# ChuhanZhou/News_Recommendation_Model

Measured on AMD Instinct MI355X. Metric: train impressions/sec, higher is better.
Workload: dtype f32

## Files before the change

### include/nrm_hotpath.h

```cpp
#ifndef NRM_HOTPATH_H
#define NRM_HOTPATH_H

#ifdef __cplusplus
extern "C" {
#endif

#define NRM_ABI_VERSION 7
#define NRM_OK 0
#define NRM_EINVAL (-1)
#define NRM_ELAUNCH (-2)

typedef void* nrm_stream_t;

int nrm_abi_version(void);
const char* nrm_last_error(void);
int nrm_build_flags(void);
const char* nrm_source_digest(void);
const char* nrm_build_info(void);


#define NRM_MMA_F32 0
#define NRM_MMA_BF16 1
#define NRM_MMA_BF16X3 2
long nrm_pwattn_packed_floats(int D);
// ... 42 lines not shown
int nrm_gemm_tn_nsplit(int ncols_i, int ncols_j, int R, int mma);
int nrm_gemm_tn(const float* A, int lda, int ncols_i, const float* B, int ldb, int ncols_j, int R,
                float* ws, int ldws, float* colsum, float* zero_out, long zero_n, int mma, nrm_stream_t stream);

int nrm_slab_reduce(const float* ws, int nsplit, int nj, int ldws, int ni, float* out, long out_istride, long out_jstride,
                    float* out2, long out2_istride, long out2_jstride, float sign2,
                    const float* vec, float* vec_out, nrm_stream_t stream);
typedef struct nrm_slab_desc {
    const float* ws; int nsplit, nj, ldws, ni;
    float* out; long out_istride, out_jstride;
    float* out2; long out2_istride, out2_jstride; float sign2;
    const float* vec; float* vec_out;
} nrm_slab_desc;
int nrm_slab_reduce_multi(const nrm_slab_desc* descs, int n, nrm_stream_t stream);

int nrm_colreduce(int mode, const float* x, const float* dy, const float* mean, const float* rstd,
                  float* s0, float* s1, int R, int N, int ld, nrm_stream_t stream);
int nrm_bn_finalize(int stage, const float* s, float* out, float* running, int R, int N, float momentum, float eps,
                    nrm_stream_t stream);
int nrm_mul_bwd(const float* dy, int lddy, const float* g, int ldg, const float* e, int lde, float* dg, float* de, int ldo,
                int R, int N, nrm_stream_t stream);
int nrm_bn_apply(const float* x, const float* mean, const float* rstd, const float* gamma, const float* beta,
                 float* y, int R, int N, int ld, nrm_stream_t stream);
int nrm_bn_backward(const float* x, const float* dy, const float* mean, const float* rstd, const float* gamma,
                    const float* s0, const float* s1, const float* add, float* dx, int R, int N, int ld, int training,
                    nrm_stream_t stream);
int nrm_concat_cols(const float* const* srcs, const long* lds, const int* widths, int n, float* out, int ldo, long R,
                    nrm_stream_t stream);

int nrm_pool_bmm(const float* W, long wsb, long wsi, long wsj, const float* X, int ldx, float* out,
// ... 60 lines not shown
```

### news_recommendation_model_amd/csrc/capi.hip

```cpp
#include <stdarg.h>
#include <stdint.h>
#include <stdio.h>
#include <stdlib.h>
#include <vector>

#include "../../include/nrm_hotpath.h"
#include "pwattn.hpp"
#include "gemm.hpp"
#include "head.hpp"
#include "pool_loss.hpp"
#include "frontend.hpp"
#include "scoring.hpp"
#include "compact.hpp"

static thread_local char g_err[512] = "";

static int fail(int code, const char* fmt, ...) {
    va_list ap;
    va_start(ap, fmt);
    vsnprintf(g_err, sizeof(g_err), fmt, ap);
    va_end(ap);
    return code;
}
static int check_hip(hipError_t e, const char* what) {
// ... 338 lines not shown
    if (n == 0) return NRM_OK;
    std::vector<nrm::SlabReduceParams> ps((size_t)n);
    for (int i = 0; i < n; ++i) {
        const nrm_slab_desc& d = descs[i];
        if (!d.ws || !d.out) return fail(NRM_EINVAL, "nrm_slab_reduce_multi: entry %d: null pointer", i);
        if (d.nsplit <= 0 || d.nj <= 0 || d.ni <= 0 || d.ldws < d.ni)
            return fail(NRM_EINVAL, "nrm_slab_reduce_multi: entry %d: nsplit=%d nj=%d ni=%d ldws=%d", i, d.nsplit, d.nj, d.ni, d.ldws);
        if ((d.vec == nullptr) != (d.vec_out == nullptr)) return fail(NRM_EINVAL, "nrm_slab_reduce_multi: entry %d: vec and vec_out go together", i);
        nrm::SlabReduceParams& p = ps[(size_t)i];
        p.ws = d.ws; p.nsplit = d.nsplit; p.nj = d.nj; p.ldws = d.ldws; p.ni = d.ni; p.out = d.out; p.ors = d.out_istride; p.ocs = d.out_jstride;
        p.out2 = d.out2; p.ors2 = d.out2_istride; p.ocs2 = d.out2_jstride; p.sign2 = d.sign2; p.vec = d.vec; p.vec_out = d.vec_out;
    }
    return check_hip(nrm::slab_reduce_multi_launch(ps.data(), n, (hipStream_t)stream), "slab_reduce_multi");
}

static int check_bn(const char* fn, int R, int N, int ld) {
    if (R < 0 || N <= 0 || N % 4 || ld % 4 || ld < N) return fail(NRM_EINVAL, "%s: R=%d N=%d ld=%d (N, ld multiples of 4)", fn, R, N, ld);
    return NRM_OK;
}

int nrm_colreduce(int mode, const float* x, const float* dy, const float* mean, const float* rstd,
                  float* s0, float* s1, int R, int N, int ld, nrm_stream_t stream) {
    if (int rc = check_bn("nrm_colreduce", R, N, ld)) return rc;
    if (!x || !s0 || (mode >= 1 && !mean) || (mode == 2 && (!dy || !rstd || !s1)) || mode < 0 || mode > 2)
        return fail(NRM_EINVAL, "nrm_colreduce: bad argument for mode %d", mode);
    return check_hip(nrm::colred_launch(mode, x, dy, mean, rstd, s0, s1, R, N, ld, (hipStream_t)stream), "colreduce");
}

int nrm_bn_finalize(int stage, const float* s, float* out, float* running, int R, int N, float momentum, float eps,
                    nrm_stream_t stream) {
// ... 265 lines not shown
```

### news_recommendation_model_amd/csrc/head.hip

```cpp
#include "common.hpp"
#include "head.hpp"

namespace nrm {

template <int MODE>
__global__ __launch_bounds__(256) void colred_kernel(const float* __restrict__ x, const float* __restrict__ dy,
                                                     const float* __restrict__ mean, const float* __restrict__ rstd,
                                                     float* __restrict__ s0, float* __restrict__ s1,
                                                     int R, int N, int ld, int rpb) {
    __shared__ f32x4 red[2][8][32];
    const int tx = threadIdx.x, ty = threadIdx.y;
    const int col = blockIdx.x * 128 + 4 * tx;
    const bool cok = col < N;
    f32x4 a0 = f32x4{0.f, 0.f, 0.f, 0.f}, a1 = a0, mu = a0, rs = a0;
    if (cok && MODE >= 1) mu = *reinterpret_cast<const f32x4*>(mean + col);
    if (cok && MODE == 2) rs = *reinterpret_cast<const f32x4*>(rstd + col);
    const int r_lo = blockIdx.y * rpb, r_hi = min(R, r_lo + rpb);
    if (cok) {
        for (int r = r_lo + ty; r < r_hi; r += 8) {
            const f32x4 xv = *reinterpret_cast<const f32x4*>(x + (size_t)r * ld + col);
            if (MODE == 0) a0 += xv;
            else if (MODE == 1) { const f32x4 d = xv - mu; a0 += d * d; }
            else {
                const f32x4 g = *reinterpret_cast<const f32x4*>(dy + (size_t)r * ld + col);
// ... 240 lines not shown
    else          hipLaunchKernelGGL(small_linear_relu_fwd_kernel<float>, grid, dim3(256), 0, st, (const float*)x, w, b, y, R, K, N, ldy);
    return hipGetLastError();
}

hipError_t small_linear_relu_bwd_launch(const void* x, int x_is_f64, const float* w, const float* b, const float* dy, int lddy,
                                        long R, int K, int N, float* dwb, hipStream_t st) {
    if (R <= 0) return hipSuccess;
    if (K < 1 || K > SL_KMAX || N < 1 || N > SL_NMAX || lddy < N) return hipErrorInvalidValue;
    long blocks = (R + 255) / 256;
    if (blocks > 256) blocks = 256;
    if (x_is_f64) hipLaunchKernelGGL(small_linear_relu_bwd_kernel<double>, dim3((unsigned)blocks), dim3(256), 0, st, (const double*)x, w, b, dy, lddy, R, K, N, dwb);
    else          hipLaunchKernelGGL(small_linear_relu_bwd_kernel<float>, dim3((unsigned)blocks), dim3(256), 0, st, (const float*)x, w, b, dy, lddy, R, K, N, dwb);
    return hipGetLastError();
}

}
```

### news_recommendation_model_amd/csrc/head.hpp

```cpp
#pragma once
#include <hip/hip_runtime.h>

namespace nrm {
hipError_t colred_launch(int mode, const float* x, const float* dy, const float* mean, const float* rstd,
                         float* s0, float* s1, int R, int N, int ld, hipStream_t st);
hipError_t bn_apply_launch(const float* x, const float* mean, const float* rstd, const float* gamma, const float* beta,
                           float* y, long R, int N, int ld, hipStream_t st);
hipError_t bn_bwd_launch(const float* x, const float* dy, const float* mean, const float* rstd, const float* gamma,
                         const float* s0, const float* s1, const float* add, float* dx, long R, int N, int ld, int training,
                         hipStream_t st);
constexpr int CONCAT_MAX = 8;
struct ConcatTable { const float* src[CONCAT_MAX]; long ld[CONCAT_MAX]; int start[CONCAT_MAX]; int n; };
hipError_t concat_cols_launch(const ConcatTable& tab, float* out, long R, int ldo, int total, hipStream_t st);
hipError_t bn_finalize_launch(int stage, const float* s, float* out, float* running, int R, int N, float momentum, float eps,
                              hipStream_t st);
hipError_t mul_bwd_launch(const float* dy, const float* g, const float* e, float* dg, float* de, long R, int N,
                          int lddy, int ldg, int lde, int ldo, hipStream_t st);
hipError_t small_linear_relu_fwd_launch(const void* x, int x_is_f64, const float* w, const float* b, float* y, long R, int K, int N,
                                        int ldy, hipStream_t st);
hipError_t small_linear_relu_bwd_launch(const void* x, int x_is_f64, const float* w, const float* b, const float* dy, int lddy,
                                        long R, int K, int N, float* dwb, hipStream_t st);
}
```

### news_recommendation_model_amd/modules.py

```python
from __future__ import annotations

import os

import torch
import torch.nn as nn
import torch.nn.functional as F

from . import ops
from .config import Dims, TIME_TABLE_ROWS, model_config

_ACTIVATIONS = {
    "relu": nn.ReLU, "gelu": nn.GELU, "tanh": nn.Tanh, "sigmoid": nn.Sigmoid,
    "leaky_relu": nn.LeakyReLU, "elu": nn.ELU,
}


class MLP(nn.Module):

    def __init__(self, input_dim, output_dim, activation_type="gelu"):
        super().__init__()
        self.fc1 = nn.Linear(input_dim, input_dim // 4)
        self.fc2 = nn.Linear(input_dim // 4, output_dim)
        self.activation_type = activation_type
        self.activation = _ACTIVATIONS.get(str(activation_type).lower(), nn.GELU)()
# ... 158 lines not shown
class UserModel(nn.Module):

    def __init__(self, user_num=0):
        super().__init__()
        self.invariant_interest_model = UserInvariantInterestModel()
        self.instant_interest_model = UserInstantInterestModel(8)
        width = (sum(self.invariant_interest_model.embed_setting) + model_config["pca_vector"]) * 2 \
            + self.instant_interest_model.output_dim
        self.bn = nn.BatchNorm1d(width)
        self.gate = MLP(width, width)
        self.mlp = MLP(width, width)
        self.out_mlp = MLP(width, 1)
        self.delta = nn.Parameter(torch.zeros(user_num + 1))
        self.bce_loss = nn.BCELoss()
        self.softmax = nn.Softmax(dim=1)

    def forward(self, x_history, x_target, x_global):
        inv = self.invariant_interest_model
        if type(inv) is UserInvariantInterestModel and not (inv._forward_hooks or inv._forward_pre_hooks):
            pooled_lab, pooled_ti, lab_t, ti_t = inv.forward_parts(x_history, x_target)
            eu_L = self.instant_interest_model(x_global)
            e = ops.concat_last((pooled_lab, pooled_ti, eu_L, lab_t, ti_t))
        else:
            eu_H, ec = inv(x_history, x_target)
            eu_L = self.instant_interest_model(x_global)
            e = ops.concat_last((eu_H, eu_L, ec))
        B, T, N = e.shape
        rows = e.reshape(B * T, N)
        g = self.gate
        if isinstance(g.activation, nn.GELU) and g.activation.approximate == "none":
            gated = ops.gate_block(rows, self.bn, g.fc1.weight, g.fc1.bias, g.fc2.weight, g.fc2.bias)
        else:
            gated = g.forward_times(ops.batch_norm(rows, self.bn), rows)
        return self.out_mlp(self.mlp(gated)).reshape(B, T)

    def forward_compact(self, x_history, xt_compact, xg_compact, plan):
        if self.training:
            raise RuntimeError("UserModel.forward_compact is inference only: call .eval() first (training-mode BatchNorm takes its "
                               "statistics over the rows of the launch, and the compact path drops the padded ones)")
        inv = self.invariant_interest_model
        ops._require_gpu(x_history, xt_compact, xg_compact)
        B, H, N = x_history.shape[0], x_history.shape[1], xt_compact.shape[0]
        if plan.B != B or plan.N != N or xg_compact.shape[0] != N:
            raise RuntimeError(f"forward_compact: plan for {plan.B} impressions / {plan.N} rows, got {B} / {N} target and {xg_compact.shape[0]} global rows")
        if B * H == 0 or N == 0:
            raise RuntimeError("cannot reshape tensor of 0 elements (empty batch / history / candidate list)")
        for att in (inv.label_attention, inv.text_img_attention):
            mlp = getattr(att, "mlp", None)
            if not (type(att) is PointwiseAttentionExpanded and isinstance(mlp, MLP) and isinstance(mlp.activation, nn.GELU)
# ... 8 lines not shown
            lab_h, ti_h = ops.frontend(x_history, True, d.n_subcat, d.pca_vector, *tables)
            lab_t, ti_t = ops.frontend(xt_compact.unsqueeze(0), False, d.n_subcat, d.pca_vector, *tables)
            lab_h = ops.linear(lab_h, inv.w1.weight, inv.w1.bias)
            pooled = []
            for att, t, h in ((inv.label_attention, lab_t[0], lab_h), (inv.text_img_attention, ti_t[0], ti_h)):
                m = att.mlp
                pooled.append(ops.attend_pool_ragged(t, h, m.fc1.weight, m.fc1.bias, m.fc2.weight, m.fc2.bias, tabs["cand_imp"],
                                                     tabs["cand_off"], plan.max_count, mma=att.mma))
            eu_L = self.instant_interest_model(xg_compact)
            rows = ops.concat_last((pooled[0], pooled[1], eu_L, lab_t[0], ti_t[0]))
            g = self.gate
            if isinstance(g.activation, nn.GELU) and g.activation.approximate == "none":
                gated = ops.gate_block(rows, self.bn, g.fc1.weight, g.fc1.bias, g.fc2.weight, g.fc2.bias)
            else:
                gated = g.forward_times(ops.batch_norm(rows, self.bn), rows)
            return self.out_mlp(self.mlp(gated)).reshape(N)

    def loss(self, id, out, label, alpha=0.95):
        return ops.softmax_bce_loss(out, self.delta, label, id, alpha)
```

### news_recommendation_model_amd/native.py

```python
from __future__ import annotations

import ctypes
import os
import threading

_HERE = os.path.dirname(os.path.abspath(__file__))
LIB_PATH = os.environ.get("NRM_HOTPATH_LIB") or os.path.join(_HERE, "libnrm_hotpath.so")
ABI_VERSION = 7

_c_fp = ctypes.c_void_p
_c_i, _c_l = ctypes.c_int, ctypes.c_long

SIGNATURES = {
    "nrm_abi_version": (_c_i, []),
    "nrm_last_error": (ctypes.c_char_p, []),
    "nrm_build_flags": (_c_i, []),
    "nrm_source_digest": (ctypes.c_char_p, []),
    "nrm_build_info": (ctypes.c_char_p, []),
    "nrm_pwattn_packed_floats": (_c_l, [_c_i]),
    "nrm_pwattn_pack_wp": (_c_i, [_c_fp, _c_i, _c_i, _c_i, _c_fp, _c_fp]),
    "nrm_pwattn_fwd": (_c_i, [_c_fp] * 9 + [_c_i] * 5 + [_c_fp]),
    "nrm_pwattn_bwd_dz": (_c_i, [_c_fp] * 7 + [_c_i] * 5 + [_c_fp]),
    "nrm_pwattn_bwd_rw_supported": (_c_i, [_c_i, _c_i]),
    "nrm_pwattn_bwd_rw_packed_floats": (_c_l, [_c_i, _c_i]),
# ... 5 lines not shown
    "nrm_pwattn_bwd_dp_dtdh": (_c_i, [_c_fp] * 6 + [_c_i] * 4 + [_c_fp]),
    "nrm_pwattn_bwd_nsplit": (_c_i, [_c_i] * 5),
    "nrm_pwattn_bwd_contract": (_c_i, [_c_fp] * 4 + [_c_i] + [_c_fp] * 3 + [_c_i] * 7 + [_c_fp]),
    "nrm_gemm_packed_floats": (_c_l, [_c_i, _c_i, _c_i]),
    "nrm_gemm_nt_bf16_supported": (_c_i, [_c_i, _c_i, _c_i]),
    "nrm_gemm_pack": (_c_i, [_c_fp, _c_l, _c_l, _c_i, _c_i, _c_fp, _c_fp]),
    "nrm_gemm_nt": (_c_i, [_c_fp, _c_i, _c_i, _c_fp, _c_i, _c_i, _c_fp, _c_fp, _c_i, _c_fp, _c_i, _c_fp, _c_i, _c_i, _c_i, _c_fp]),
    "nrm_slab_reduce": (_c_i, [_c_fp, _c_i, _c_i, _c_i, _c_i, _c_fp, _c_l, _c_l, _c_fp, _c_l, _c_l, ctypes.c_float,
                               _c_fp, _c_fp, _c_fp]),
    "nrm_bn_finalize": (_c_i, [_c_i, _c_fp, _c_fp, _c_fp, _c_i, _c_i, ctypes.c_float, ctypes.c_float, _c_fp]),
    "nrm_mul_bwd": (_c_i, [_c_fp, _c_i, _c_fp, _c_i, _c_fp, _c_i, _c_fp, _c_fp, _c_i, _c_i, _c_i, _c_fp]),
    "nrm_gemm_tn_nsplit": (_c_i, [_c_i, _c_i, _c_i, _c_i]),
    "nrm_gemm_tn": (_c_i, [_c_fp, _c_i, _c_i, _c_fp, _c_i, _c_i, _c_i, _c_fp, _c_i, _c_fp, _c_fp, _c_l, _c_i, _c_fp]),
    "nrm_gemm_pack_multi": (_c_i, [_c_fp, _c_i, _c_fp]),
    "nrm_slab_reduce_multi": (_c_i, [_c_fp, _c_i, _c_fp]),
    "nrm_colreduce": (_c_i, [_c_i] + [_c_fp] * 6 + [_c_i] * 3 + [_c_fp]),
    "nrm_bn_apply": (_c_i, [_c_fp] * 6 + [_c_i] * 3 + [_c_fp]),
    "nrm_bn_backward": (_c_i, [_c_fp] * 9 + [_c_i] * 4 + [_c_fp]),
    "nrm_concat_cols": (_c_i, [_c_fp, _c_fp, _c_fp, _c_i, _c_fp, _c_i, _c_l, _c_fp]),
    "nrm_pool_bmm": (_c_i, [_c_fp, _c_l, _c_l, _c_l, _c_fp, _c_i, _c_fp] + [_c_i] * 5 + [_c_fp]),
    "nrm_pool_rowdot": (_c_i, [_c_fp, _c_i, _c_fp, _c_fp] + [_c_i] * 4 + [_c_fp, _c_i, _c_fp]),
    "nrm_small_linear_relu_fwd": (_c_i, [_c_fp, _c_i, _c_fp, _c_fp, _c_fp, _c_l, _c_i, _c_i, _c_i, _c_fp]),
    "nrm_small_linear_relu_bwd": (_c_i, [_c_fp, _c_i, _c_fp, _c_fp, _c_fp, _c_i, _c_l, _c_i, _c_i, _c_fp, _c_fp]),
    "nrm_loss_fwd_bwd": (_c_i, [_c_fp, _c_i, _c_fp, _c_i, _c_fp, _c_fp, _c_l, ctypes.c_float, _c_i, _c_i, _c_fp, _c_fp, _c_i, _c_fp, _c_fp, _c_fp]),
    "nrm_adam_step": (_c_i, [_c_fp] * 4 + [_c_l] + [ctypes.c_float] * 5 + [_c_i, _c_i, _c_fp]),
    "nrm_adam_step_dev": (_c_i, [_c_fp] * 4 + [_c_l] + [ctypes.c_float] * 5 + [_c_fp, _c_i, _c_fp]),
    "nrm_gather_flat": (_c_i, [_c_fp, _c_fp, _c_fp, _c_i, _c_fp, _c_l, _c_fp]),
    "nrm_row_auc": (_c_i, [_c_fp] * 3 + [_c_i, _c_i] + [_c_fp] * 3),
    "nrm_ensemble_rank_max_candidates": (_c_i, []),
    "nrm_ensemble_rank": (_c_i, [_c_fp] * 3 + [_c_i, _c_fp, _c_fp, _c_i, _c_i] + [_c_fp] * 5),
# ... 97 lines not shown
```

### news_recommendation_model_amd/ops.py

```python
from __future__ import annotations

import torch

from . import native

EPI_BIAS, EPI_GELU, EPI_DGELU, EPI_MUL = 0, 1, 2, 3
MMA_F32, MMA_BF16, MMA_BF16X3 = 0, 1, 2
DZ_F32, DZ_HL4 = 0, 1
_MMA_NAMES = {"f32": MMA_F32, "fp32": MMA_F32, "float32": MMA_F32, "bf16": MMA_BF16, "bfloat16": MMA_BF16, "bf16x3": MMA_BF16X3}
_default_mma = MMA_F32


def resolve_mma(mma):
    if mma is None:
        return _default_mma
    if isinstance(mma, str):
        if mma.lower() not in _MMA_NAMES:
            raise ValueError(f"attention arithmetic {mma!r}: expected 'f32', 'bf16' or 'bf16x3'")
        return _MMA_NAMES[mma.lower()]
    if int(mma) not in (MMA_F32, MMA_BF16, MMA_BF16X3):
        raise ValueError(f"attention arithmetic {mma!r}: expected NRM_MMA_F32 (0), NRM_MMA_BF16 (1) or NRM_MMA_BF16X3 (2)")
    return int(mma)


# ... 109 lines not shown
    return ctypes.cast(ctypes.pointer(desc_or_array), ctypes.c_void_p)


def repack_persistent(owners=None):
    _packs.epoch += 1
    mine = None if owners is None else {id(o) for o in owners}
    live = []
    for key, ent in list(_packs.entries.items()):
        owner = ent.owner()
        if owner is None or owner.data_ptr() != ent.owner_ptr:
            _packs.entries.pop(key, None)
            continue
        if mine is not None and id(owner) not in mine:
            continue
        live.append((ent, owner))
    if not live:
        return 0
    arr = (native.PackDesc * len(live))(*[_pack_desc_of(ent, owner) for ent, owner in live])
    native.call("nrm_gemm_pack_multi", _ctypes_ref(arr), len(live), native.stream_ptr())
    for ent, owner in live:
        ent.version, ent.epoch = owner._version, _packs.epoch
    return len(live)


def invalidate_packed_weights():
    _packs.entries.clear()
    _packs.epoch += 1
    _packs.generation += 1


def packed_weights_generation():
    return _packs.generation


_flop_meter = None


def flop_meter_start():
    global _flop_meter
    _flop_meter = {"dense": 0.0, "contraction": 0.0, "dense_launches": 0, "contraction_launches": 0}

# ... 10 lines not shown
        _flop_meter[kind + "_launches"] += 1


import os as _os
_FORCE_F32_GEMM = _os.environ.get("NRM_GEMM_F32") == "1"


def _dense_mma(M, K, mma):
    mma = _default_dense_mma if mma is None else mma
    if _FORCE_F32_GEMM or (mma != MMA_F32 and not native.load().nrm_gemm_nt_bf16_supported(int(M), int(K), int(mma))):
        return MMA_F32
    return mma


def _gemm_nt(x, w_src, row_stride, col_stride, n_out, k_red, bias, epilogue, z=None, m=None, src2=None, sign2=0.0, owner=None,
             mma=None):
    st = native.stream_ptr()
    M = x.shape[0]
    mma = _dense_mma(M, k_red, mma)
    packed = _pack(w_src, row_stride, col_stride, n_out, k_red, src2, sign2, owner, mma)
    ldy = _pad4(n_out)
    y = torch.empty(M, ldy, dtype=torch.float32, device=x.device)
    if epilogue in (EPI_GELU, EPI_MUL):
        z = torch.empty(M, ldy, dtype=torch.float32, device=x.device)
    _count_flops("dense", 2.0 * M * n_out * k_red)
    native.call("nrm_gemm_nt", native.ptr(x), x.stride(0), M, native.ptr(packed), n_out, k_red,
                native.ptr(bias) if bias is not None else None, native.ptr(y), ldy,
                native.ptr(z) if z is not None else None, z.stride(0) if z is not None else 0,
                native.ptr(m) if m is not None else None, m.stride(0) if m is not None else 0, epilogue, mma, st)
    return y[:, :n_out], (z[:, :n_out] if epilogue in (EPI_GELU, EPI_MUL) else None)


def _gemm_tn_slabs(a, b, want_colsum, zero_out=None, mma=None):
    lib = native.load()
    R, ni = a.shape
# ... 21 lines not shown
        self.prev, _deferred["on"] = _deferred["on"], True
        return self

    def __exit__(self, *exc):
        _deferred["on"] = self.prev
        if exc[0] is not None:
            _deferred["pending"].clear()
        return False


def verify_deferred_targets(params):
    pend = _deferred["pending"]
    if not pend:
        return
    by_ptr = {p.data_ptr(): p for p in params}
    for rec in pend:
        p = by_ptr.get(rec["target"])
        if p is None or not p.requires_grad:
            continue
        if p.grad is None or p.grad.untyped_storage().data_ptr() != rec["keep"][0].data_ptr():
            _deferred["pending"] = []
            _join_wgrad_stream()
            raise RuntimeError(
                "deferred slab reductions: a weight gradient was copied or accumulated before its reduction ran (a weight "
                "used more than once in the graph, a gradient that existed before backward(), a gradient hook, or "
                "create_graph): its values would be wrong. Run this backward outside ops.deferred_slab_reductions() -- "
                "trainer.train_step(..., defer_reductions=False).")


def flush_slab_reductions():
    pend, _deferred["pending"] = _deferred["pending"], []
    _join_wgrad_stream()
    if not pend:
        return
    descs = (native.SlabDesc * len(pend))()
    for d, rec in zip(descs, pend):
        d.ws, d.nsplit, d.nj, d.ldws, d.ni = rec["ws"].data_ptr(), rec["nsplit"], rec["nj"], rec["ldws"], rec["ni"]
        d.out, d.out_istride, d.out_jstride = rec["out"], rec["out_is"], rec["out_js"]
        d.out2, d.out2_istride, d.out2_jstride, d.sign2 = rec["out2"], rec["out2_is"], rec["out2_js"], rec["sign2"]
        if rec["vec"] is not None:
            d.vec, d.vec_out = rec["vec"].data_ptr(), rec["vec_out"]
    native.call("nrm_slab_reduce_multi", descs, len(pend), native.stream_ptr())


def _slab_reduce(ws, nsplit, nj, ldws, ni, out, out_is, out_js, out2=None, out2_is=0, out2_js=0, sign2=0.0,
                 vec=None, vec_out=None, target=None):
    if _deferred["on"]:
        _deferred["pending"].append(dict(
            ws=ws, nsplit=nsplit, nj=nj, ldws=ldws, ni=ni, out=out.data_ptr(), out_is=out_is, out_js=out_js,
            out2=out2.data_ptr() if out2 is not None else None, out2_is=out2_is, out2_js=out2_js, sign2=float(sign2),
            vec=vec, vec_out=vec_out.data_ptr() if vec_out is not None else None,
            target=target.data_ptr() if target is not None else None,
            keep=(out.untyped_storage(), out2.untyped_storage() if out2 is not None else None,
                  vec_out.untyped_storage() if vec_out is not None else None)))
        return
    native.call("nrm_slab_reduce", native.ptr(ws), nsplit, nj, ldws, ni, native.ptr(out), out_is, out_js,
                native.ptr(out2) if out2 is not None else None, out2_is, out2_js, float(sign2),
# ... 560 lines not shown

torch.library.register_autograd("nrm::mlp_gelu_fwd", _mlp_backward, setup_context=_mlp_setup, lib=_LIB)


def mlp_gelu(x, fc1_weight, fc1_bias, fc2_weight, fc2_bias, mul=None):
    lead = x.shape[:-1]
    if x.numel() == 0 and x.shape[-1] == fc1_weight.shape[1]:
        out = _degenerate((*lead, fc2_weight.shape[0]), x, fc1_weight, fc1_bias, fc2_weight, fc2_bias)
        return out if mul is None else out * mul
    _require_gpu(x, fc1_weight, fc2_weight)
    m2 = mul.reshape(-1, mul.shape[-1]) if mul is not None else None
    y = mlp_gelu_fwd(x.reshape(-1, x.shape[-1]), fc1_weight, fc1_bias, fc2_weight, fc2_bias, m2)[0]
    return y.reshape(*lead, fc2_weight.shape[0])


def _bn_stats_impl(x, running_mean, running_var, momentum, eps):
    _require_gpu(x, running_mean, running_var)
    x = _rows(x)
    R, N = x.shape
    ld = x.stride(0)
    st = native.stream_ptr()
    dev = x.device
    s = torch.zeros(2, N, dtype=torch.float32, device=dev)
    mean = torch.empty(N, dtype=torch.float32, device=dev)
    rstd = torch.empty(N, dtype=torch.float32, device=dev)
    native.call("nrm_colreduce", 0, native.ptr(x), None, None, None, native.ptr(s[0]), None, R, N, ld, st)
    native.call("nrm_bn_finalize", 0, native.ptr(s[0]), native.ptr(mean), native.ptr(running_mean), R, N, float(momentum), float(eps), st)
    native.call("nrm_colreduce", 1, native.ptr(x), None, native.ptr(mean), None, native.ptr(s[1]), None, R, N, ld, st)
    native.call("nrm_bn_finalize", 1, native.ptr(s[1]), native.ptr(rstd), native.ptr(running_var), R, N, float(momentum), float(eps), st)
    return mean, rstd
# ... 841 lines not shown
ensemble_rank_ragged = _op("ensemble_rank_ragged", "(Tensor[] logits, Tensor cand_off, Tensor pad_mult, Tensor? label, int T) -> "
                           "(Tensor score, Tensor rank, Tensor live, Tensor metrics)", _ensemble_rank_ragged_impl, _ensemble_rank_ragged_fake)


def _adam_step_impl(param, grad, exp_avg, exp_avg_sq, state, lr, beta1, beta2, eps, weight_decay, zero_grad):
    _require_gpu(param, grad, exp_avg, exp_avg_sq, state)
    native.call("nrm_adam_step_dev", native.ptr(param), native.ptr(grad), native.ptr(exp_avg), native.ptr(exp_avg_sq),
                param.numel(), float(lr), float(beta1), float(beta2), float(eps), float(weight_decay), native.ptr(state),
                1 if zero_grad else 0, native.stream_ptr())


adam_step = _op("adam_step", "(Tensor(a!) param, Tensor(b!) grad, Tensor(c!) exp_avg, Tensor(d!) exp_avg_sq, Tensor(e!) state, "
                "float lr, float beta1, float beta2, float eps, float weight_decay, bool zero_grad) -> ()",
                _adam_step_impl, lambda *a: None)

OPS = ("pwattn_fwd", "pwattn_bwd", "linear_fwd", "linear_bwd", "small_linear_relu_fwd", "small_linear_relu_bwd", "mlp_gelu_fwd", "mlp_gelu_bwd", "batch_norm_stats", "batch_norm_apply",
       "batch_norm_bwd", "gate_block_fwd", "gate_block_bwd", "concat_cols",
       "weighted_pool_fwd", "weighted_pool_bwd", "attend_pool_fwd", "attend_pool_bwd", "softmax_bce_loss", "frontend_fwd", "frontend_bwd",
       "frontend_pair_fwd", "frontend_pair_bwd", "row_auc", "ensemble_rank", "compact_gather", "attend_pool_ragged_fwd", "ensemble_rank_ragged",
       "adam_step")
```

Baseline: 33490.

## Fold consecutive linear layers of head MLPs into one precomputed weight

The linear pair mlp.fc2 followed by out_mlp.fc1 has no nonlinearity between them, so their weights are multiplied into one folded matrix and bias. A fused kernel builds the packed forward and backward GEMM images in one pass, and a backward kernel splits the folded-weight gradient back into gradients for the two original weights and biases, possibly deferred onto the wgrad stream. This removes one per-row GEMM and one activation buffer in both forward and backward. In exchange it adds per-step refold and split GEMMs on the weights, forces the f32 MMA path for the folded GEMMs, and changes rounding order.

```diff
diff --git a/include/nrm_hotpath.h b/include/nrm_hotpath.h
--- a/include/nrm_hotpath.h
+++ b/include/nrm_hotpath.h
@@ -80,6 +80,11 @@
 } nrm_slab_desc;
 int nrm_slab_reduce_multi(const nrm_slab_desc* descs, int n, nrm_stream_t stream);
 
+int nrm_head_fold(const float* w_o1, const float* b_o1, const float* w_m2, const float* b_m2, int P, int Q, int R,
+                  float* packed_fwd, float* packed_bwd, float* bias, nrm_stream_t stream);
+int nrm_head_fold_bwd(const float* dwp, int ldp, const float* dbp, const float* w_o1, const float* w_m2, const float* b_m2,
+                      int P, int Q, int R, float* dw_o1, float* dw_m2, float* db_o1, float* db_m2, nrm_stream_t stream);
+
 int nrm_colreduce(int mode, const float* x, const float* dy, const float* mean, const float* rstd,
                   float* s0, float* s1, int R, int N, int ld, nrm_stream_t stream);
 int nrm_bn_finalize(int stage, const float* s, float* out, float* running, int R, int N, float momentum, float eps,
diff --git a/news_recommendation_model_amd/csrc/capi.hip b/news_recommendation_model_amd/csrc/capi.hip
--- a/news_recommendation_model_amd/csrc/capi.hip
+++ b/news_recommendation_model_amd/csrc/capi.hip
@@ -376,6 +376,29 @@
     return check_hip(nrm::slab_reduce_multi_launch(ps.data(), n, (hipStream_t)stream), "slab_reduce_multi");
 }
 
+int nrm_head_fold(const float* w_o1, const float* b_o1, const float* w_m2, const float* b_m2, int P, int Q, int R,
+                  float* packed_fwd, float* packed_bwd, float* bias, nrm_stream_t stream) {
+    if (!w_o1 || !w_m2 || !packed_fwd || !packed_bwd || !bias) return fail(NRM_EINVAL, "nrm_head_fold: null pointer");
+    if (P <= 0 || Q <= 0 || R <= 0 || Q % 4 || !al16(w_o1))
+        return fail(NRM_EINVAL, "nrm_head_fold: P=%d Q=%d R=%d (Q a multiple of 4, w_o1 16-byte aligned)", P, Q, R);
+    const nrm::GemmNtPlan pf = nrm::gemm_nt_plan(P), pb = nrm::gemm_nt_plan(R);
+    nrm::HeadFoldParams p = {};
+    p.wo = w_o1; p.wm = w_m2; p.bo = b_o1; p.bm = b_m2; p.img_f = packed_fwd; p.img_b = packed_bwd; p.bias = bias;
+    p.P = P; p.Q = Q; p.R = R; p.rows_f = pf.rows; p.kch_f = (R + 15) / 16; p.rows_b = pb.rows; p.kch_b = (P + 15) / 16;
+    return check_hip(nrm::head_fold_launch(p, (hipStream_t)stream), "head_fold");
+}
+
+int nrm_head_fold_bwd(const float* dwp, int ldp, const float* dbp, const float* w_o1, const float* w_m2, const float* b_m2,
+                      int P, int Q, int R, float* dw_o1, float* dw_m2, float* db_o1, float* db_m2, nrm_stream_t stream) {
+    if (!dwp || !dbp || !w_o1 || !w_m2) return fail(NRM_EINVAL, "nrm_head_fold_bwd: null pointer");
+    if (P <= 0 || Q <= 0 || R <= 0 || ldp % 4 || ldp < R || !al16(dwp))
+        return fail(NRM_EINVAL, "nrm_head_fold_bwd: P=%d Q=%d R=%d ldp=%d (ldp a multiple of 4 covering R, 16-byte aligned rows)", P, Q, R, ldp);
+    nrm::HeadSplitParams p = {};
+    p.dwp = dwp; p.ldp = ldp; p.dbp = dbp; p.wo = w_o1; p.wm = w_m2; p.bm = b_m2; p.dwo = dw_o1; p.dwm = dw_m2; p.dbo = db_o1; p.dbm = db_m2;
+    p.P = P; p.Q = Q; p.R = R;
+    return check_hip(nrm::head_fold_bwd_launch(p, (hipStream_t)stream), "head_fold_bwd");
+}
+
 static int check_bn(const char* fn, int R, int N, int ld) {
     if (R < 0 || N <= 0 || N % 4 || ld % 4 || ld < N) return fail(NRM_EINVAL, "%s: R=%d N=%d ld=%d (N, ld multiples of 4)", fn, R, N, ld);
     return NRM_OK;
diff --git a/news_recommendation_model_amd/csrc/head.hip b/news_recommendation_model_amd/csrc/head.hip
--- a/news_recommendation_model_amd/csrc/head.hip
+++ b/news_recommendation_model_amd/csrc/head.hip
@@ -278,4 +278,158 @@
     return hipGetLastError();
 }
 
-}
+__global__ __launch_bounds__(256) void head_fold_kernel(const HeadFoldParams p) {
+#if defined(__HIP_DEVICE_COMPILE__)
+    __shared__ float part[4][16][17];
+    __shared__ float bpart[4][16];
+    const int tid = threadIdx.x;
+    const int lane = tid & 63;
+    const int wave = __builtin_amdgcn_readfirstlane(tid >> 6);
+    const int r16 = lane & 15, q = lane >> 4;
+    const int ti = blockIdx.x % p.ti, tj = blockIdx.x / p.ti;
+    const int i0 = ti * 16, j0 = tj * 16;
+    f32x4 acc = f32x4{0.f, 0.f, 0.f, 0.f};
+    float bs = 0.f;
+    if (i0 < p.P && j0 < p.R) {
+        const int nch = (p.Q + 15) >> 4;
+        const int i = i0 + r16, j = j0 + r16;
+        const bool iok = i < p.P, jok = j < p.R;
+        const float* arow = p.wo + (size_t)(iok ? i : 0) * p.Q;
+        const bool want_b = tj == 0 && p.bm != nullptr;
+        for (int c = wave; c < nch; c += 16) {
+            f32x4 a[4];
+            float b[4][4];
+#pragma unroll
+            for (int u = 0; u < 4; ++u) {
+                const int k = 16 * (c + 4 * u) + 4 * q;
+                a[u] = f32x4{0.f, 0.f, 0.f, 0.f};
+                if (iok && k < p.Q) a[u] = *reinterpret_cast<const f32x4*>(arow + k);
+#pragma unroll
+                for (int e = 0; e < 4; ++e) b[u][e] = (jok && k + e < p.Q) ? p.wm[(size_t)(k + e) * p.R + j] : 0.f;
+            }
+#pragma unroll
+            for (int u = 0; u < 4; ++u) {
+#pragma unroll
+                for (int e = 0; e < 4; ++e) acc = mfma16(a[u][e], b[u][e], acc);
+                const int k = 16 * (c + 4 * u) + 4 * q;
+                if (want_b && iok && k < p.Q) {
+#pragma unroll
+                    for (int e = 0; e < 4; ++e) bs = fmaf(a[u][e], p.bm[k + e], bs);
+                }
+            }
+        }
+    }
+#pragma unroll
+    for (int e = 0; e < 4; ++e) part[wave][4 * q + e][r16] = acc[e];
+    bs = sum_rows4(bs);
+    if (q == 0) bpart[wave][r16] = bs;
+    __syncthreads();
+    const int a = tid >> 4, b = tid & 15;
+    float v = (part[0][a][b] + part[1][a][b]) + (part[2][a][b] + part[3][a][b]);
+    if (i0 + a >= p.P || j0 + b >= p.R) v = 0.f;
+    part[0][a][b] = v;
+    __syncthreads();
+    {
+        const int row = i0 + a;
+        if (row < p.rows_f && tj < p.kch_f)
+            p.img_f[((size_t)tj * p.rows_f + row) * 16 + 4 * ((b >> 2) ^ swz4(row)) + (b & 3)] = v;
+    }
+    {
+        const int row = j0 + a;
+        if (row < p.rows_b && ti < p.kch_b)
+            p.img_b[((size_t)ti * p.rows_b + row) * 16 + 4 * ((b >> 2) ^ swz4(row)) + (b & 3)] = part[0][b][a];
+    }
+    if (tj == 0 && tid < 16 && i0 + tid < p.P)
+        p.bias[i0 + tid] = ((bpart[0][tid] + bpart[1][tid]) + (bpart[2][tid] + bpart[3][tid])) + (p.bo ? p.bo[i0 + tid] : 0.f);
+#endif
+}
+
+hipError_t head_fold_launch(HeadFoldParams p, hipStream_t st) {
+    p.ti = p.rows_f / 16;
+    p.tj = p.rows_b / 16;
+    if (p.ti < p.kch_b || p.tj < p.kch_f) return hipErrorInvalidValue;
+    hipLaunchKernelGGL(head_fold_kernel, dim3((unsigned)(p.ti * p.tj)), dim3(256), 0, st, p);
+    return hipGetLastError();
+}
+
+__global__ __launch_bounds__(256) void head_fold_bwd_kernel(const HeadSplitParams p) {
+#if defined(__HIP_DEVICE_COMPILE__)
+    const int tid = threadIdx.x;
+    const int lane = tid & 63;
+    const int wave = __builtin_amdgcn_readfirstlane(tid >> 6);
+    const int r16 = lane & 15, q = lane >> 4;
+    if ((int)blockIdx.x >= p.mm_blocks) {
+        const int c = ((int)blockIdx.x - p.mm_blocks) * 256 + tid;
+        if (p.dbm && c < p.Q) {
+            float s = 0.f;
+#pragma unroll 4
+            for (int i = 0; i < p.P; ++i) s = fmaf(p.wo[(size_t)i * p.Q + c], p.dbp[i], s);
+            p.dbm[c] = s;
+        }
+        if (p.dbo && c < p.P) p.dbo[c] = p.dbp[c];
+        return;
+    }
+    const int id = blockIdx.x * 4 + wave;
+    if (id >= p.na + p.nb) return;
+    f32x4 acc = f32x4{0.f, 0.f, 0.f, 0.f};
+    const int tq = (p.Q + 15) >> 4, tr = (p.R + 15) >> 4;
+    if (id < p.na) {
+        const int c0 = (id % tq) * 16, i0 = (id / tq) * 16;
+        const int i = i0 + r16, c = c0 + r16;
+        const bool iok = i < p.P, cok = c < p.Q;
+        const float* arow = p.dwp + (size_t)(iok ? i : 0) * p.ldp;
+        const float* brow = p.wm + (size_t)(cok ? c : 0) * p.R;
+        for (int k0 = 0; k0 < p.R; k0 += 16) {
+            const int k = k0 + 4 * q;
+            f32x4 a = f32x4{0.f, 0.f, 0.f, 0.f};
+            float b[4];
+            if (iok && k < p.R) a = *reinterpret_cast<const f32x4*>(arow + k);
+#pragma unroll
+            for (int e = 0; e < 4; ++e) {
+                const bool kok = k + e < p.R;
+                a[e] = kok ? a[e] : 0.f;
+                b[e] = (cok && kok) ? brow[k + e] : 0.f;
+            }
+#pragma unroll
+            for (int e = 0; e < 4; ++e) acc = mfma16(a[e], b[e], acc);
+        }
+        const float bmc = (p.bm && cok) ? p.bm[c] : 0.f;
+#pragma unroll
+        for (int e = 0; e < 4; ++e)
+            if (i0 + 4 * q + e < p.P && cok) p.dwo[(size_t)(i0 + 4 * q + e) * p.Q + c] = fmaf(p.dbp[i0 + 4 * q + e], bmc, acc[e]);
+    } else {
+        const int t = id - p.na;
+        const int j0 = (t % tr) * 16, c0 = (t / tr) * 16;
+        const int c = c0 + r16, j = j0 + r16;
+        const bool cok = c < p.Q, jok = j < p.R;
+        for (int k0 = 0; k0 < p.P; k0 += 16) {
+            const int k = k0 + 4 * q;
+            float a[4], b[4];
+#pragma unroll
+            for (int e = 0; e < 4; ++e) {
+                const bool kok = k + e < p.P;
+                a[e] = (cok && kok) ? p.wo[(size_t)(k + e) * p.Q + c] : 0.f;
+                b[e] = (jok && kok) ? p.dwp[(size_t)(k + e) * p.ldp + j] : 0.f;
+            }
+#pragma unroll
+            for (int e = 0; e < 4; ++e) acc = mfma16(a[e], b[e], acc);
+        }
+#pragma unroll
+        for (int e = 0; e < 4; ++e)
+            if (c0 + 4 * q + e < p.Q && jok) p.dwm[(size_t)(c0 + 4 * q + e) * p.R + j] = acc[e];
+    }
+#endif
+}
+
+hipError_t head_fold_bwd_launch(HeadSplitParams p, hipStream_t st) {
+    const int tp = (p.P + 15) / 16, tq = (p.Q + 15) / 16, tr = (p.R + 15) / 16;
+    p.na = p.dwo ? tp * tq : 0;
+    p.nb = p.dwm ? tq * tr : 0;
+    p.mm_blocks = (p.na + p.nb + 3) / 4;
+    const int nv = (p.dbm || p.dbo) ? ((p.Q > p.P ? p.Q : p.P) + 255) / 256 : 0;
+    if (p.mm_blocks + nv == 0) return hipSuccess;
+    hipLaunchKernelGGL(head_fold_bwd_kernel, dim3((unsigned)(p.mm_blocks + nv)), dim3(256), 0, st, p);
+    return hipGetLastError();
+}
+
+}
diff --git a/news_recommendation_model_amd/csrc/head.hpp b/news_recommendation_model_amd/csrc/head.hpp
--- a/news_recommendation_model_amd/csrc/head.hpp
+++ b/news_recommendation_model_amd/csrc/head.hpp
@@ -20,4 +20,24 @@
                                         int ldy, hipStream_t st);
 hipError_t small_linear_relu_bwd_launch(const void* x, int x_is_f64, const float* w, const float* b, const float* dy, int lddy,
                                         long R, int K, int N, float* dwb, hipStream_t st);
+struct HeadFoldParams {
+    const float* wo; const float* wm;
+    const float* bo; const float* bm;
+    float* img_f; float* img_b;
+    float* bias;
+    int P, Q, R;
+    int rows_f, kch_f, rows_b, kch_b;
+    int ti, tj;
+};
+hipError_t head_fold_launch(HeadFoldParams p, hipStream_t st);
+struct HeadSplitParams {
+    const float* dwp; int ldp;
+    const float* dbp;
+    const float* wo; const float* wm;
+    const float* bm;
+    float* dwo; float* dwm; float* dbo; float* dbm;
+    int P, Q, R;
+    int na, nb, mm_blocks;
+};
+hipError_t head_fold_bwd_launch(HeadSplitParams p, hipStream_t st);
 }
diff --git a/news_recommendation_model_amd/modules.py b/news_recommendation_model_amd/modules.py
--- a/news_recommendation_model_amd/modules.py
+++ b/news_recommendation_model_amd/modules.py
@@ -196,6 +196,27 @@
         self.delta = nn.Parameter(torch.zeros(user_num + 1))
         self.bce_loss = nn.BCELoss()
         self.softmax = nn.Softmax(dim=1)
+
+    def _tail(self, gated):
+        if gated.dim() == 2 and gated.shape[0] > 0 and self.head_fold_applies(gated.shape[1]):
+            m, o = self.mlp, self.out_mlp
+            return ops.head_tail(gated, m.fc1.weight, m.fc1.bias, m.fc2.weight, m.fc2.bias, o.fc1.weight, o.fc1.bias,
+                                 o.fc2.weight, o.fc2.bias)
+        return self.out_mlp(self.mlp(gated))
+
+    def head_fold_applies(self, width):
+        if not ops.head_fold_enabled():
+            return False
+        for mod in (self.mlp, self.out_mlp):
+            if type(mod) is not MLP or type(mod.fc1) is not nn.Linear or type(mod.fc2) is not nn.Linear:
+                return False
+            if not isinstance(mod.activation, nn.GELU) or mod.activation.approximate != "none":
+                return False
+            for layer in (mod, mod.fc1, mod.fc2, mod.activation):
+                if layer._forward_hooks or layer._forward_pre_hooks or layer._backward_hooks or layer._backward_pre_hooks:
+                    return False
+        m, o = self.mlp, self.out_mlp
+        return ops.head_fold_shapes_ok(width, m.fc1.weight, m.fc2.weight, m.fc2.bias, o.fc1.weight, o.fc1.bias, o.fc2.weight)
 
     def forward(self, x_history, x_target, x_global):
         inv = self.invariant_interest_model
@@ -214,7 +235,7 @@
             gated = ops.gate_block(rows, self.bn, g.fc1.weight, g.fc1.bias, g.fc2.weight, g.fc2.bias)
         else:
             gated = g.forward_times(ops.batch_norm(rows, self.bn), rows)
-        return self.out_mlp(self.mlp(gated)).reshape(B, T)
+        return self._tail(gated).reshape(B, T)
 
     def forward_compact(self, x_history, xt_compact, xg_compact, plan):
         if self.training:
@@ -253,7 +274,7 @@
                 gated = ops.gate_block(rows, self.bn, g.fc1.weight, g.fc1.bias, g.fc2.weight, g.fc2.bias)
             else:
                 gated = g.forward_times(ops.batch_norm(rows, self.bn), rows)
-            return self.out_mlp(self.mlp(gated)).reshape(N)
+            return self._tail(gated).reshape(N)
 
     def loss(self, id, out, label, alpha=0.95):
         return ops.softmax_bce_loss(out, self.delta, label, id, alpha)
diff --git a/news_recommendation_model_amd/native.py b/news_recommendation_model_amd/native.py
--- a/news_recommendation_model_amd/native.py
+++ b/news_recommendation_model_amd/native.py
@@ -43,6 +43,8 @@
     "nrm_gemm_tn": (_c_i, [_c_fp, _c_i, _c_i, _c_fp, _c_i, _c_i, _c_i, _c_fp, _c_i, _c_fp, _c_fp, _c_l, _c_i, _c_fp]),
     "nrm_gemm_pack_multi": (_c_i, [_c_fp, _c_i, _c_fp]),
     "nrm_slab_reduce_multi": (_c_i, [_c_fp, _c_i, _c_fp]),
+    "nrm_head_fold": (_c_i, [_c_fp] * 4 + [_c_i] * 3 + [_c_fp] * 4),
+    "nrm_head_fold_bwd": (_c_i, [_c_fp, _c_i, _c_fp, _c_fp, _c_fp, _c_fp, _c_i, _c_i, _c_i] + [_c_fp] * 5),
     "nrm_colreduce": (_c_i, [_c_i] + [_c_fp] * 6 + [_c_i] * 3 + [_c_fp]),
     "nrm_bn_apply": (_c_i, [_c_fp] * 6 + [_c_i] * 3 + [_c_fp]),
     "nrm_bn_backward": (_c_i, [_c_fp] * 9 + [_c_i] * 4 + [_c_fp]),
diff --git a/news_recommendation_model_amd/ops.py b/news_recommendation_model_amd/ops.py
--- a/news_recommendation_model_amd/ops.py
+++ b/news_recommendation_model_amd/ops.py
@@ -147,17 +147,18 @@
         if mine is not None and id(owner) not in mine:
             continue
         live.append((ent, owner))
-    if not live:
-        return 0
-    arr = (native.PackDesc * len(live))(*[_pack_desc_of(ent, owner) for ent, owner in live])
-    native.call("nrm_gemm_pack_multi", _ctypes_ref(arr), len(live), native.stream_ptr())
-    for ent, owner in live:
-        ent.version, ent.epoch = owner._version, _packs.epoch
+    if live:
+        arr = (native.PackDesc * len(live))(*[_pack_desc_of(ent, owner) for ent, owner in live])
+        native.call("nrm_gemm_pack_multi", _ctypes_ref(arr), len(live), native.stream_ptr())
+        for ent, owner in live:
+            ent.version, ent.epoch = owner._version, _packs.epoch
+    _refold_persistent(mine)
     return len(live)
 
 
 def invalidate_packed_weights():
     _packs.entries.clear()
+    _folds.clear()
     _packs.epoch += 1
     _packs.generation += 1
 
@@ -198,11 +199,14 @@
 
 
 def _gemm_nt(x, w_src, row_stride, col_stride, n_out, k_red, bias, epilogue, z=None, m=None, src2=None, sign2=0.0, owner=None,
-             mma=None):
+             mma=None, packed=None):
     st = native.stream_ptr()
     M = x.shape[0]
-    mma = _dense_mma(M, k_red, mma)
-    packed = _pack(w_src, row_stride, col_stride, n_out, k_red, src2, sign2, owner, mma)
+    if packed is not None:
+        mma = MMA_F32
+    else:
+        mma = _dense_mma(M, k_red, mma)
+        packed = _pack(w_src, row_stride, col_stride, n_out, k_red, src2, sign2, owner, mma)
     ldy = _pad4(n_out)
     y = torch.empty(M, ldy, dtype=torch.float32, device=x.device)
     if epilogue in (EPI_GELU, EPI_MUL):
@@ -254,11 +258,16 @@
     if not pend:
         return
     by_ptr = {p.data_ptr(): p for p in params}
+    targets = []
     for rec in pend:
-        p = by_ptr.get(rec["target"])
+        targets.append((rec["target"], rec["keep"][0]))
+        if rec.get("post") is not None:
+            targets.extend(rec["post"]["targets"])
+    for target, storage in targets:
+        p = by_ptr.get(target)
         if p is None or not p.requires_grad:
             continue
-        if p.grad is None or p.grad.untyped_storage().data_ptr() != rec["keep"][0].data_ptr():
+        if p.grad is None or p.grad.untyped_storage().data_ptr() != storage.data_ptr():
             _deferred["pending"] = []
             _join_wgrad_stream()
             raise RuntimeError(
@@ -281,6 +290,9 @@
         if rec["vec"] is not None:
             d.vec, d.vec_out = rec["vec"].data_ptr(), rec["vec_out"]
     native.call("nrm_slab_reduce_multi", descs, len(pend), native.stream_ptr())
+    for rec in pend:
+        if rec.get("post") is not None:
+            _head_fold_split(rec["post"])
 
 
 def _slab_reduce(ws, nsplit, nj, ldws, ni, out, out_is, out_js, out2=None, out2_is=0, out2_js=0, sign2=0.0,
@@ -871,6 +883,215 @@
     return y.reshape(*lead, fc2_weight.shape[0])
 
 
+class _FoldEntry:
+    __slots__ = ("img_f", "img_b", "bias", "owners", "ptrs", "versions", "epoch", "dims")
+
+
+_folds = {}
+
+
+def head_fold_enabled():
+    return _os.environ.get("NRM_HEAD_FOLD") != "0" and _default_dense_mma == MMA_F32
+
+
+def _fold_launch(ent, wo, bo, wm, bm):
+    P, Q, R = ent.dims
+    _count_flops("dense", 2.0 * P * Q * R)
+    native.call("nrm_head_fold", native.ptr(wo), native.ptr(bo) if bo is not None else None, native.ptr(wm),
+                native.ptr(bm) if bm is not None else None, P, Q, R, native.ptr(ent.img_f), native.ptr(ent.img_b),
+                native.ptr(ent.bias), native.stream_ptr())
+    ent.versions = tuple(t._version for t in (wo, bo, wm, bm) if t is not None)
+    ent.epoch = _packs.epoch
+
+
+def _fold_owners(ent):
+    ts = tuple(r() if r is not None else None for r in ent.owners)
+    for t, r, ptr in zip(ts, ent.owners, ent.ptrs):
+        if r is not None and (t is None or t.data_ptr() != ptr):
+            return None
+    return ts
+
+
+def _head_fold_image(wo, bo, wm, bm):
+    import weakref
+    ts = (wo, bo, wm, bm)
+    key = tuple(t.data_ptr() if t is not None else 0 for t in ts)
+    ent = _folds.get(key)
+    if ent is not None:
+        live = _fold_owners(ent)
+        if live is None or any(a is not b for a, b in zip(live, ts)):
+            ent = None
+    if ent is not None and ent.epoch == _packs.epoch and ent.versions == tuple(t._version for t in ts if t is not None):
+        return ent
+    if ent is None:
+        lib = native.load()
+        (P, Q), R = wo.shape, wm.shape[1]
+        ent = _FoldEntry()
+        ent.dims = (int(P), int(Q), int(R))
+        ent.img_f = torch.empty(lib.nrm_gemm_packed_floats(P, R, MMA_F32), dtype=torch.float32, device=wo.device)
+        ent.img_b = torch.empty(lib.nrm_gemm_packed_floats(R, P, MMA_F32), dtype=torch.float32, device=wo.device)
+        ent.bias = torch.zeros(_pad4(P), dtype=torch.float32, device=wo.device)
+        ent.owners = tuple(weakref.ref(t) if t is not None else None for t in ts)
+        ent.ptrs = key
+        _folds[key] = ent
+        for t in (wo, wm):
+            weakref.finalize(t, _drop_fold, key, id(ent))
+    _fold_launch(ent, *ts)
+    return ent
+
+
+def _drop_fold(key, ident):
+    if id(_folds.get(key)) == ident:
+        _folds.pop(key, None)
+
+
+def _refold_persistent(mine):
+    for key, ent in list(_folds.items()):
+        ts = _fold_owners(ent)
+        if ts is None:
+            _folds.pop(key, None)
+            continue
+        if mine is not None and not all(id(t) in mine for t in ts if t is not None):
+            continue
+        _fold_launch(ent, *ts)
+
+
+def _head_fold_split(rec):
+    P, Q, R = rec["dims"]
+    _count_flops("dense", 2.0 * P * Q * R * ((rec["dwo"] is not None) + (rec["dwm"] is not None)))
+    import ctypes
+    c = lambda v: ctypes.c_void_p(v) if v is not None else None
+    native.call("nrm_head_fold_bwd", native.ptr(rec["dwp"]), rec["dwp"].stride(0), native.ptr(rec["dbp"]), native.ptr(rec["wo"]),
+                native.ptr(rec["wm"]), native.ptr(rec["bm"]) if rec["bm"] is not None else None, P, Q, R, c(rec["dwo"]), c(rec["dwm"]), c(rec["dbo"]), c(rec["dbm"]), native.stream_ptr())
+
+
+def _head_fold_grads(dz2, a1, wo, bo, wm, bm, need_wo, need_bo, need_wm, need_bm):
+    (P, Q), R = wo.shape, wm.shape[1]
+    dev = dz2.device
+    f = lambda *shape: torch.empty(shape, dtype=torch.float32, device=dev)
+    out = (f(P, Q) if need_wo else None, f(P) if need_bo else None, f(Q, R) if need_wm else None, f(Q) if need_bm else None)
+    ctx = _wgrad_stream(dz2, a1)
+    with ctx as side:
+        dwp = f(P, _pad4(R))
+        ws, cs, nsplit, ldws = _gemm_tn_slabs(dz2, a1, True, zero_out=dwp, mma=MMA_F32)
+        dbp = f(P)
+        _slab_reduce(ws, nsplit, R, ldws, P, dwp, dwp.stride(0), 1, vec=cs, vec_out=dbp)
+        if side:
+            for t in (dwp, ws, cs, dbp):
+                t.record_stream(ctx.main)
+    rec = dict(dims=(int(P), int(Q), int(R)), dwp=dwp, dbp=dbp, wo=wo, wm=wm, bm=bm,
+               **{k: (t.data_ptr() if t is not None else None) for k, t in zip(("dwo", "dbo", "dwm", "dbm"), out)})
+    if _deferred["on"]:
+        rec["keep"] = tuple(t.untyped_storage() for t in out if t is not None)
+        rec["targets"] = [(p.data_ptr(), t.untyped_storage()) for p, t in zip((wo, bo, wm, bm), out) if p is not None and t is not None]
+        _deferred["pending"][-1]["post"] = rec
+    else:
+        _head_fold_split(rec)
+    return out
+
+
+def _head_tail_fwd_impl(x, w1, b1, wm, bm, wo, bo, w3, b3):
+    _require_gpu(x, w1, wm, wo, w3)
+    x = _rows(x)
+    o1, o3 = w1, w3
+    w1, w3 = _f32c(w1), _f32c(w3)
+    o1, o3 = (w1 if w1 is o1 else None), (w3 if w3 is o3 else None)
+    (N1, K1), (Q, R), (P, Q2), (N3, K3) = w1.shape, wm.shape, wo.shape, w3.shape
+    if x.shape[1] != K1 or R != N1 or Q2 != Q or K3 != P:
+        raise RuntimeError(f"head tail: input has {x.shape[1]} features; layers {K1}->{N1}, {R}->{Q}, {Q2}->{P}, {K3}->{N3} do not chain")
+    a1, z1 = _gemm_nt(x, w1, K1, 1, N1, K1, _f32c(b1) if b1 is not None else None, EPI_GELU, owner=o1)
+    ent = _head_fold_image(wo, bo, wm, bm)
+    a2, z2 = _gemm_nt(a1, None, 0, 0, P, R, ent.bias, EPI_GELU, packed=ent.img_f)
+    y, _ = _gemm_nt(a2, w3, K3, 1, N3, K3, _f32c(b3) if b3 is not None else None, EPI_BIAS, owner=o3)
+    return y, a1, z1, a2, z2
+
+
+def _head_tail_fwd_fake(x, w1, b1, wm, bm, wo, bo, w3, b3):
+    M, N1, P, N3 = x.shape[0], w1.shape[0], wo.shape[0], w3.shape[0]
+    return (_padded_empty(x, M, N3), _padded_empty(x, M, N1), _padded_empty(x, M, N1), _padded_empty(x, M, P), _padded_empty(x, M, P))
+
+
+head_tail_fwd = _op("head_tail_fwd", "(Tensor x, Tensor w1, Tensor? b1, Tensor wm, Tensor? bm, Tensor wo, Tensor? bo, Tensor w3, Tensor? b3) "
+                    "-> (Tensor, Tensor, Tensor, Tensor, Tensor)", _head_tail_fwd_impl, _head_tail_fwd_fake)
+
+
+def _head_tail_bwd_impl(dy, x, w1, wm, bm, wo, bo, w3, a1, z1, a2, z2, has_b1, has_b3, need_dx, need_wm, need_bm, need_wo, need_bo):
+    _require_gpu(dy, x, w1, wm, wo, w3)
+    o1, o3 = w1, w3
+    p1, p3 = w1, w3
+    x, w1, w3 = _rows(x), _f32c(w1), _f32c(w3)
+    o1, o3 = (w1 if w1 is o1 else None), (w3 if w3 is o3 else None)
+    (N1, K1), (Q, R), P, (N3, K3) = w1.shape, wm.shape, wo.shape[0], w3.shape
+    dy = _rows(dy)
+    dev = x.device
+    e = lambda: torch.empty((0,), dtype=torch.float32, device=dev)
+    dw3, db3 = _gemm_tn(dy, a2, has_b3, target=p3)
+    dz2, _ = _gemm_nt(dy, w3, 1, K3, K3, N3, None, EPI_DGELU, z=z2, owner=o3)
+    dwo = dbo = dwm = dbm = None
+    if need_wm or need_bm or need_wo or need_bo:
+        dwo, dbo, dwm, dbm = _head_fold_grads(dz2, a1, wo, bo, wm, bm, need_wo, need_bo, need_wm, need_bm)
+    ent = _head_fold_image(wo, bo, wm, bm)
+    dz1, _ = _gemm_nt(dz2, None, 0, 0, R, P, None, EPI_DGELU, z=z1, packed=ent.img_b)
+    dw1, db1 = _gemm_tn(dz1, x, has_b1, target=p1)
+    dx = _gemm_nt(dz1, w1, 1, K1, K1, N1, None, EPI_BIAS, owner=o1)[0] if need_dx else e()
+    opt = lambda t: t if t is not None else e()
+    return dx, dw1, (db1 if has_b1 else e()), opt(dwm), opt(dbm), opt(dwo), opt(dbo), dw3, (db3 if has_b3 else e())
+
+
+def _head_tail_bwd_fake(dy, x, w1, wm, bm, wo, bo, w3, a1, z1, a2, z2, has_b1, has_b3, need_dx, need_wm, need_bm, need_wo, need_bo):
+    M, (N1, K1), (Q, R), P, (N3, K3) = x.shape[0], w1.shape, wm.shape, wo.shape[0], w3.shape
+    f = lambda *shape: x.new_empty(shape, dtype=torch.float32)
+    return (_padded_empty(x, M, K1) if need_dx else f(0), f(N1, K1), f(N1) if has_b1 else f(0), f(Q, R) if need_wm else f(0),
+            f(Q) if need_bm else f(0), f(P, Q) if need_wo else f(0), f(P) if need_bo else f(0), f(N3, K3), f(N3) if has_b3 else f(0))
+
+
+head_tail_bwd = _op("head_tail_bwd", "(Tensor dy, Tensor x, Tensor w1, Tensor wm, Tensor? bm, Tensor wo, Tensor? bo, Tensor w3, Tensor a1, "
+                    "Tensor z1, Tensor a2, Tensor z2, bool has_b1, bool has_b3, bool need_dx, bool need_wm, bool need_bm, bool need_wo, "
+                    "bool need_bo) -> (Tensor, Tensor, Tensor, Tensor, Tensor, Tensor, Tensor, Tensor, Tensor)",
+                    _head_tail_bwd_impl, _head_tail_bwd_fake)
+
+
+def _head_tail_setup(ctx, inputs, output):
+    x, w1, b1, wm, bm, wo, bo, w3, b3 = inputs
+    y, a1, z1, a2, z2 = output
+    ctx.set_materialize_grads(False)
+    ctx.has = (b1 is not None, bm is not None, bo is not None, b3 is not None)
+    ctx.save_for_backward(x, w1, wm, wo, w3, a1, z1, a2, z2, *[b for b in (bm, bo) if b is not None])
+
+
+def _head_tail_backward(ctx, dy, _da1, _dz1, _da2, _dz2):
+    if dy is None:
+        return (None,) * 9
+    x, w1, wm, wo, w3, a1, z1, a2, z2, *rest = ctx.saved_tensors
+    has_b1, has_bm, has_bo, has_b3 = ctx.has
+    bm = rest.pop(0) if has_bm else None
+    bo = rest.pop(0) if has_bo else None
+    need = ctx.needs_input_grad
+    need_wm, need_bm, need_wo, need_bo = need[3], has_bm and need[4], need[5], has_bo and need[6]
+    dx, dw1, db1, dwm, dbm, dwo, dbo, dw3, db3 = head_tail_bwd(dy, x, w1, wm, bm, wo, bo, w3, a1, z1, a2, z2, has_b1, has_b3, need[0],
+                                                               need_wm, need_bm, need_wo, need_bo)
+    return ((dx if need[0] else None), dw1, (db1 if has_b1 else None), (dwm if need_wm else None), (dbm if need_bm else None),
+            (dwo if need_wo else None), (dbo if need_bo else None), dw3, (db3 if has_b3 else None))
+
+
+torch.library.register_autograd("nrm::head_tail_fwd", _head_tail_backward, setup_context=_head_tail_setup, lib=_LIB)
+
+
+def head_fold_shapes_ok(x_cols, w1, wm, bm, wo, bo, w3):
+    ts = (w1, wm, bm, wo, bo, w3)
+    if any(t is None or t.dtype != torch.float32 or not t.is_contiguous() for t in ts):
+        return False
+    if w1.dim() != 2 or wm.dim() != 2 or wo.dim() != 2 or w3.dim() != 2:
+        return False
+    return (x_cols == w1.shape[1] and x_cols % 4 == 0 and wm.shape[1] == w1.shape[0] and wo.shape[1] == wm.shape[0]
+            and wm.shape[0] % 4 == 0 and w3.shape[1] == wo.shape[0] and bm.shape[0] == wm.shape[0] and bo.shape[0] == wo.shape[0])
+
+
+def head_tail(x, w1, b1, wm, bm, wo, bo, w3, b3):
+    _require_gpu(x, w1, wm, wo, w3)
+    return head_tail_fwd(x, w1, b1, wm, bm, wo, bo, w3, b3)[0]
+
+
 def _bn_stats_impl(x, running_mean, running_var, momentum, eps):
     _require_gpu(x, running_mean, running_var)
     x = _rows(x)
@@ -1742,7 +1963,7 @@
                 "float lr, float beta1, float beta2, float eps, float weight_decay, bool zero_grad) -> ()",
                 _adam_step_impl, lambda *a: None)
 
-OPS = ("pwattn_fwd", "pwattn_bwd", "linear_fwd", "linear_bwd", "small_linear_relu_fwd", "small_linear_relu_bwd", "mlp_gelu_fwd", "mlp_gelu_bwd", "batch_norm_stats", "batch_norm_apply",
+OPS = ("pwattn_fwd", "pwattn_bwd", "head_tail_fwd", "head_tail_bwd", "linear_fwd", "linear_bwd", "small_linear_relu_fwd", "small_linear_relu_bwd", "mlp_gelu_fwd", "mlp_gelu_bwd", "batch_norm_stats", "batch_norm_apply",
        "batch_norm_bwd", "gate_block_fwd", "gate_block_bwd", "concat_cols",
        "weighted_pool_fwd", "weighted_pool_bwd", "attend_pool_fwd", "attend_pool_bwd", "softmax_bce_loss", "frontend_fwd", "frontend_bwd",
        "frontend_pair_fwd", "frontend_pair_bwd", "row_auc", "ensemble_rank", "compact_gather", "attend_pool_ragged_fwd", "ensemble_rank_ragged",
```

Measured after the change: 35340, median of 6. 1.06x the previous value.
